# tensorflow/adanet

Measured on NVIDIA H100. Metric: candidate-train examples/sec per AdaNet iteration, higher is better.
Workload: dtype f32

## Files before the change

### adanet_b200/csrc/planes.cu

```cuda
#include <cuda.h>
#include <cudaTypedefs.h>

#include <stdlib.h>
#include <string.h>

#include <algorithm>
#include <atomic>
#include <mutex>
#include <string>
#include <unordered_map>
#include <vector>

#include "dense_simt.cuh"
#include "planes.cuh"
#include "wgmma.cuh"

namespace adn {
namespace pl {

static constexpr int BM = 128, BN = 64;
static constexpr int STAGES = 3;
static constexpr int A_TILE = BM * 128;
static constexpr int B_TILE = BN * 128;
static constexpr int STAGE_BYTES = 2 * A_TILE + 2 * B_TILE;
static constexpr int CONSUMERS = 2;
static constexpr int CONSUMER_WARPS = 4 * CONSUMERS;
static constexpr int EPI_WARPS = 4;
static constexpr int NUM_THREADS = 128 * (1 + CONSUMERS) + 32 * EPI_WARPS;
static constexpr int PRODUCER_REGS = 40, EPI_REGS = 136, CONSUMER_REGS = 168;
static_assert(128 * (PRODUCER_REGS + EPI_REGS) + 128 * CONSUMERS * CONSUMER_REGS <= 65536, "register file");
static_assert(PRODUCER_REGS < 65536 / NUM_THREADS && EPI_REGS > 65536 / NUM_THREADS &&
              CONSUMER_REGS > 65536 / NUM_THREADS, "setmaxnreg.dec / .inc");
static constexpr int ACC_BUFS = 2;
static constexpr int ACC_TILE_FLOATS = BM * BN;
static constexpr int ACC_BYTES = ACC_BUFS * ACC_TILE_FLOATS * 4;
static constexpr int EPI_STAGE_FLOATS = 32 * 16;
static constexpr int EPI_BYTES = EPI_WARPS * 2 * EPI_STAGE_FLOATS * 4;
static constexpr int BAR_BYTES = 256;
static constexpr int SMEM_BYTES = 1024 + STAGES * STAGE_BYTES + ACC_BYTES + EPI_BYTES + BAR_BYTES;
static_assert(SMEM_BYTES <= 232448, "shared memory per block");
static constexpr int MAX_SPLITS = 64;

template <int FMT> struct Fmt;
template <> struct Fmt<FMT_TF32> {
  static constexpr int BK = 32;
  static constexpr int CHUNK = 4;
};
template <> struct Fmt<FMT_F16> {
  static constexpr int BK = 64;
  static constexpr int CHUNK = 2;
};

enum { EPI_BIAS_ACT = 0, EPI_MASK = 1, EPI_PARTIAL = 2 };

struct GemmParams {
  int M, N;
  int tiles_m, tiles_n, splits;
  int tiles;
  float inv_tiles, inv_tiles_n, inv_tiles_m;
  int total_kb;
  int kb_per_split;
  int a_mn, b_mn;
  int out_planes;
  int m_fastest;
  void* out;
  void* out_lo;
  int ldc;
  int out_nb32;
  int out_tma;
  const float* bias;
  int act;
  uint32_t* out_bits;
  const uint32_t* mask_bits;
  float* colsum_part;
  int colsum_ld;
  float out_mul;
  unsigned int* ovf;
  uint32_t drop_thresh;
  uint32_t drop_key0;
  float drop_scale;
  const int64_t* drop_step;
};

__device__ __forceinline__ uint32_t smem_u32(const void* p) { return (uint32_t)__cvta_generic_to_shared(p); }

__device__ __forceinline__ void mbar_init(uint32_t bar, uint32_t count) {
  asm volatile("mbarrier.init.shared::cta.b64 [%0], %1;" ::"r"(bar), "r"(count));
}
__device__ __forceinline__ void mbar_expect_tx(uint32_t bar, uint32_t bytes) {
  asm volatile("mbarrier.arrive.expect_tx.shared::cta.b64 _, [%0], %1;" ::"r"(bar), "r"(bytes) : "memory");
}
__device__ __forceinline__ void mbar_arrive(uint32_t bar) {
  asm volatile("mbarrier.arrive.shared::cta.b64 _, [%0];" ::"r"(bar) : "memory");
}
__device__ __forceinline__ void mbar_wait(uint32_t bar, uint32_t parity) {
  uint32_t ok = 0;
  long long t0 = 0;
  for (uint32_t it = 0;; ++it) {
    asm volatile(
        "{\n\t.reg .pred p;\n\t"
        "mbarrier.try_wait.parity.shared::cta.b64 p, [%1], %2;\n\t"
        "selp.u32 %0, 1, 0, p;\n\t}"
        : "=r"(ok)
        : "r"(bar), "r"(parity)
        : "memory");
    if (ok) return;
    if ((it & 1023u) == 1023u) {
      long long now = clock64();
      if (t0 == 0) t0 = now;
      else if (now - t0 > 4000000000LL) __trap();
    }
  }
}
__device__ __forceinline__ void tma_load_3d(const CUtensorMap* map, uint32_t bar, uint32_t dst, int c0, int c1, int c2) {
  asm volatile(
      "cp.async.bulk.tensor.3d.shared::cluster.global.mbarrier::complete_tx::bytes [%0], [%1, {%3, %4, %5}], [%2];"
      ::"r"(dst), "l"(reinterpret_cast<uint64_t>(map)), "r"(bar), "r"(c0), "r"(c1), "r"(c2)
      : "memory");
}
__device__ __forceinline__ void tma_store_3d(const CUtensorMap* map, uint32_t src, int c0, int c1, int c2) {
  asm volatile("cp.async.bulk.tensor.3d.global.shared::cta.bulk_group [%0, {%2, %3, %4}], [%1];"
               ::"l"(reinterpret_cast<uint64_t>(map)), "r"(src), "r"(c0), "r"(c1), "r"(c2)
               : "memory");
}
__device__ __forceinline__ void bulk_commit() { asm volatile("cp.async.bulk.commit_group;" ::: "memory"); }
__device__ __forceinline__ void bulk_wait_read0() { asm volatile("cp.async.bulk.wait_group.read 0;" ::: "memory"); }
__device__ __forceinline__ void bulk_wait_read1() { asm volatile("cp.async.bulk.wait_group.read 1;" ::: "memory"); }
__device__ __forceinline__ void bulk_wait0() { asm volatile("cp.async.bulk.wait_group 0;" ::: "memory"); }
__device__ __forceinline__ void fence_async_smem() { asm volatile("fence.proxy.async.shared::cta;" ::: "memory"); }
__device__ __forceinline__ void sts_v4(uint32_t addr, uint32_t a, uint32_t b, uint32_t c, uint32_t d) {
  asm volatile("st.shared.v4.b32 [%0], {%1, %2, %3, %4};" ::"r"(addr), "r"(a), "r"(b), "r"(c), "r"(d) : "memory");
}
__device__ __forceinline__ void tma_prefetch_desc(const CUtensorMap* map) {
  asm volatile("prefetch.tensormap [%0];" ::"l"(reinterpret_cast<uint64_t>(map)) : "memory");
}

struct Item {
  int m0, n0, kb0, nkb, split;
};
__device__ __forceinline__ int fast_div(int n, float inv) { return (int)(((float)n + 0.5f) * inv); }

__device__ __forceinline__ Item decode_item(const GemmParams& g, int item) {
  Item it;
  it.split = (g.splits == 1) ? 0 : fast_div(item, g.inv_tiles);
  const int t = item - it.split * g.tiles;
  if (g.m_fastest) {
    const int tn = fast_div(t, g.inv_tiles_m);
    it.n0 = tn * BN;
    it.m0 = (t - tn * g.tiles_m) * BM;
  } else {
    const int tm = (g.tiles_n == 1) ? t : fast_div(t, g.inv_tiles_n);
    it.m0 = tm * BM;
    it.n0 = (t - tm * g.tiles_n) * BN;
  }
  it.kb0 = it.split * g.kb_per_split;
  it.nkb = min(g.total_kb, it.kb0 + g.kb_per_split) - it.kb0;
  return it;
}

__device__ __forceinline__ uint32_t pack_h2(__half a, __half b) {
  return (uint32_t)__half_as_ushort(a) | ((uint32_t)__half_as_ushort(b) << 16);
}

__device__ __forceinline__ void st_global_v8(void* p, const uint32_t (&w)[8]) {
  uint4* q = reinterpret_cast<uint4*>(p);
  q[0] = make_uint4(w[0], w[1], w[2], w[3]);
  q[1] = make_uint4(w[4], w[5], w[6], w[7]);
}

template <int FMT>
__device__ __forceinline__ void store_row32_planes(const GemmParams& g, const float* a, int my_row, int cbase) {
  constexpr int BK = Fmt<FMT>::BK;
  const size_t poff = ((size_t)(cbase / BK) * g.M + my_row) * BK + (cbase % BK);
  if (FMT == FMT_F16) {
    uint32_t hw[16], lw[16];
#pragma unroll
    for (int q = 0; q < 16; ++q) {
      const __half2 h2 = __floats2half2_rn(a[2 * q], a[2 * q + 1]);
      const float2 hf = __half22float2(h2);
      const __half2 l2 = __floats2half2_rn((a[2 * q] - hf.x) * 2048.0f, (a[2 * q + 1] - hf.y) * 2048.0f);
      hw[q] = *reinterpret_cast<const uint32_t*>(&h2);
      lw[q] = *reinterpret_cast<const uint32_t*>(&l2);
    }
    __half* hp = reinterpret_cast<__half*>(g.out) + poff;
    __half* lp = reinterpret_cast<__half*>(g.out_lo) + poff;
    st_global_v8(hp, reinterpret_cast<const uint32_t(&)[8]>(hw[0]));
    st_global_v8(hp + 16, reinterpret_cast<const uint32_t(&)[8]>(hw[8]));
    st_global_v8(lp, reinterpret_cast<const uint32_t(&)[8]>(lw[0]));
    st_global_v8(lp + 16, reinterpret_cast<const uint32_t(&)[8]>(lw[8]));
  } else {
    uint32_t hw[32], lw[32];
#pragma unroll
    for (int j = 0; j < 32; ++j) {
      float h, l;
// ... 244 lines not shown
              *reinterpret_cast<float4*>(op) = make_float4(v[0], v[1], v[2], v[3]);
            } else {
#pragma unroll
              for (int k = 0; k < 4; ++k)
                if (col + k < g.N) op[k] = v[k];
            }
          }
        }
      }
      if (EPI == EPI_MASK && g.colsum_part) {
#pragma unroll
        for (int k = 0; k < 4; ++k) {
          cs[k] += __shfl_xor_sync(0xffffffffu, cs[k], 4);
          cs[k] += __shfl_xor_sync(0xffffffffu, cs[k], 8);
          cs[k] += __shfl_xor_sync(0xffffffffu, cs[k], 16);
        }
        if (rsub == 0) {
          float* cp = g.colsum_part + (size_t)(mrow0 >> 5) * g.colsum_ld + col;
#pragma unroll
          for (int k = 0; k < 4; ++k)
            if (col + k < g.colsum_ld) cp[k] = cs[k];
        }
      }
    }
    __syncwarp();
  }
#undef ADN_SWZ
}

static constexpr int MAX_GROUP = 8;

struct alignas(64) Problem {
  CUtensorMap a_hi, a_lo, b_hi, b_lo;
  CUtensorMap o_hi, o_lo;
  GemmParams g;
  int item0;
  int pad_[3];
};
struct alignas(64) Group {
  Problem p[MAX_GROUP];
  int n;
  int total_items;
};

__device__ __forceinline__ int find_problem(const Group& grp, int cur, int item, int& next0) {
  while (item >= next0) {
    ++cur;
    next0 = (cur + 1 < grp.n) ? grp.p[cur + 1].item0 : 0x7fffffff;
  }
  return cur;
}
__device__ __forceinline__ int first_next0(const Group& grp) { return grp.n > 1 ? grp.p[1].item0 : 0x7fffffff; }

struct EpiItem {
  int p;
  Item it;
  uint32_t mw0, mw1;
  uint32_t drop_step;
};
template <int EPI>
__device__ __forceinline__ EpiItem epi_fetch(const Group& grp, int& cur, int& next0, int item, int tile_row) {
  EpiItem e;
  cur = find_problem(grp, cur, item, next0);
  e.p = cur;
  const GemmParams& g = grp.p[cur].g;
  e.it = decode_item(g, item - grp.p[cur].item0);
  e.mw0 = e.mw1 = 0xffffffffu;
  if (EPI == EPI_MASK && g.mask_bits) {
    const int my_row = e.it.m0 + tile_row, kbo = e.it.n0 >> 5;
    const bool row_ok = my_row < g.M;
    e.mw0 = (row_ok && kbo < g.out_nb32) ? __ldg(g.mask_bits + (size_t)kbo * g.M + my_row) : 0u;
    e.mw1 = (row_ok && kbo + 1 < g.out_nb32) ? __ldg(g.mask_bits + (size_t)(kbo + 1) * g.M + my_row) : 0u;
  }
  e.drop_step = (EPI == EPI_BIAS_ACT && g.drop_thresh != 0u) ? (uint32_t)(*g.drop_step) : 0u;
  return e;
}

template <int R> __device__ __forceinline__ void setmaxnreg_inc() { asm volatile("setmaxnreg.inc.sync.aligned.u32 %0;" ::"n"(R)); }
template <int R> __device__ __forceinline__ void setmaxnreg_dec() { asm volatile("setmaxnreg.dec.sync.aligned.u32 %0;" ::"n"(R)); }

__device__ __forceinline__ int acc_off(int row, int col) {
  return row * BN + ((((col >> 2) ^ row) & 7) | ((col >> 2) & 8)) * 4 + (col & 3);
}

template <int FMT>
__device__ __forceinline__ void fold_chunk(float (&acc)[32], const float (&H)[32], const float (&S)[32]) {
#pragma unroll
  for (int j = 0; j < 32; ++j) acc[j] += H[j];
  if (FMT == FMT_F16) {
#pragma unroll
    for (int j = 0; j < 32; ++j) acc[j] = fmaf(S[j], 1.0f / 2048.0f, acc[j]);
  } else {
#pragma unroll
    for (int j = 0; j < 32; ++j) acc[j] += S[j];
  }
}

template <int A_MN, int B_MN>
__device__ __forceinline__ void f16_kblock(uint32_t st, int wgi, float (&H)[32], float (&S)[32], bool first) {
  const uint32_t a_hi = st + (uint32_t)wgi * 8192u, a_lo = a_hi + A_TILE;
  const uint32_t b_hi = st + 2 * A_TILE, b_lo = b_hi + B_TILE;
  constexpr uint32_t a_step = A_MN ? 2048u : 32u, b_step = B_MN ? 2048u : 32u;
#pragma unroll
  for (int k = 0; k < 4; ++k) {
    const uint32_t sd = (first && k == 0) ? 0u : 1u;
    const uint64_t dah = wg::desc_sw128(a_hi + k * a_step), dal = wg::desc_sw128(a_lo + k * a_step);
    const uint64_t dbh = wg::desc_sw128(b_hi + k * b_step), dbl = wg::desc_sw128(b_lo + k * b_step);
    wg::mma_f16_n64<A_MN, B_MN>(H, dah, dbh, sd);
    wg::mma_f16_n64<A_MN, B_MN>(S, dah, dbl, sd);
    wg::mma_f16_n64<A_MN, B_MN>(S, dal, dbh, 1u);
  }
}

__device__ __forceinline__ uint32_t sw128_off(int r, int c) {
  return (uint32_t)(r * 128 + ((((c >> 4) ^ r) & 7) << 4) + (c & 15));
}
template <int MN>
__device__ __forceinline__ uint32_t tf32_off(int mn, int k) {
  return MN ? (uint32_t)((mn >> 5) * 4096) + sw128_off(k, 4 * (mn & 31)) : sw128_off(mn, 4 * k);
}
__device__ __forceinline__ void mma_tf32_16x8(float* d, const uint32_t (&a)[4], uint32_t b0, uint32_t b1) {
  asm volatile("mma.sync.aligned.m16n8k8.row.col.f32.tf32.tf32.f32 {%0, %1, %2, %3}, {%4, %5, %6, %7}, {%8, %9}, "
               "{%0, %1, %2, %3};"
               : "+f"(d[0]), "+f"(d[1]), "+f"(d[2]), "+f"(d[3])
               : "r"(a[0]), "r"(a[1]), "r"(a[2]), "r"(a[3]), "r"(b0), "r"(b1));
}
template <int A_MN, int B_MN>
__device__ __forceinline__ void tf32_kblock(const uint8_t* st, int arow0, int lane, float (&H)[32], float (&S)[32]) {
  const uint8_t* ah = st;
  const uint8_t* al = st + A_TILE;
  const uint8_t* bh = st + 2 * A_TILE;
  const uint8_t* bl = bh + B_TILE;
  const int gid = lane >> 2, tq = lane & 3;
#pragma unroll
  for (int ks = 0; ks < 4; ++ks) {
    uint32_t fa_h[4], fa_l[4];
#pragma unroll
    for (int e = 0; e < 4; ++e) {
      const uint32_t o = tf32_off<A_MN>(arow0 + gid + 8 * (e & 1), 8 * ks + tq + 4 * (e >> 1));
      fa_h[e] = *reinterpret_cast<const uint32_t*>(ah + o);
      fa_l[e] = *reinterpret_cast<const uint32_t*>(al + o);
    }
#pragma unroll
    for (int j = 0; j < 8; ++j) {
      const uint32_t o0 = tf32_off<B_MN>(8 * j + gid, 8 * ks + tq), o1 = tf32_off<B_MN>(8 * j + gid, 8 * ks + tq + 4);
      const uint32_t bh0 = *reinterpret_cast<const uint32_t*>(bh + o0), bh1 = *reinterpret_cast<const uint32_t*>(bh + o1);
      const uint32_t bl0 = *reinterpret_cast<const uint32_t*>(bl + o0), bl1 = *reinterpret_cast<const uint32_t*>(bl + o1);
      mma_tf32_16x8(&H[4 * j], fa_h, bh0, bh1);
      mma_tf32_16x8(&S[4 * j], fa_h, bl0, bl1);
      mma_tf32_16x8(&S[4 * j], fa_l, bh0, bh1);
    }
  }
}
template <int FMT, int EPI>
__global__ void __launch_bounds__(NUM_THREADS, 1)
pl_gemm_kernel(const __grid_constant__ Group grp) {
  constexpr int BK = Fmt<FMT>::BK;
  constexpr int CHUNK = Fmt<FMT>::CHUNK;
  constexpr int A_MN = EPI == EPI_PARTIAL, B_MN = EPI != EPI_MASK;
  extern __shared__ uint8_t smem_raw[];
  uint8_t* smem = reinterpret_cast<uint8_t*>((reinterpret_cast<uintptr_t>(smem_raw) + 1023) & ~(uintptr_t)1023);
  float* acc_stage = reinterpret_cast<float*>(smem + STAGES * STAGE_BYTES);
  float* epi_stage = reinterpret_cast<float*>(smem + STAGES * STAGE_BYTES + ACC_BYTES);
  uint64_t* bars = reinterpret_cast<uint64_t*>(smem + STAGES * STAGE_BYTES + ACC_BYTES + EPI_BYTES);
  uint64_t* full_bar = bars;
  uint64_t* empty_bar = bars + STAGES;
  uint64_t* tile_full = bars + 2 * STAGES;
  uint64_t* tile_empty = tile_full + ACC_BUFS;

  const int warp = __shfl_sync(0xffffffffu, threadIdx.x >> 5, 0);
  const int lane = threadIdx.x & 31;
  const int n_items = grp.total_items;

  if (threadIdx.x == 0) {
    for (int s = 0; s < STAGES; ++s) {
      mbar_init(smem_u32(&full_bar[s]), 1);
      mbar_init(smem_u32(&empty_bar[s]), CONSUMER_WARPS);
    }
    for (int b = 0; b < ACC_BUFS; ++b) {
      mbar_init(smem_u32(&tile_full[b]), 128 * CONSUMERS);
      mbar_init(smem_u32(&tile_empty[b]), 32 * EPI_WARPS);
    }
    asm volatile("fence.mbarrier_init.release.cluster;" ::: "memory");
  }
  if (warp == 1 && lane < grp.n) {
    tma_prefetch_desc(&grp.p[lane].a_hi);
    tma_prefetch_desc(&grp.p[lane].a_lo);
    tma_prefetch_desc(&grp.p[lane].b_hi);
    tma_prefetch_desc(&grp.p[lane].b_lo);
  }
  __syncthreads();

  if (warp < 4) {
    setmaxnreg_dec<PRODUCER_REGS>();
    if (warp == 0 && lane == 0) {
      uint32_t s = 0, ph = 0;
      int cur = 0, next0 = first_next0(grp);
      const uint32_t smem0 = smem_u32(smem);
      for (int item = blockIdx.x; item < n_items; item += gridDim.x) {
        cur = find_problem(grp, cur, item, next0);
        const Problem& pr = grp.p[cur];
        const GemmParams& g = pr.g;
        const Item it = decode_item(g, item - pr.item0);
        for (int kb = 0; kb < it.nkb; ++kb) {
          mbar_wait(smem_u32(&empty_bar[s]), ph ^ 1);
          const uint32_t fb = smem_u32(&full_bar[s]);
          mbar_expect_tx(fb, STAGE_BYTES);
          const uint32_t base = smem0 + s * STAGE_BYTES;
          const int kc = it.kb0 + kb;
          const int a1 = A_MN ? kc * BK : it.m0, a2 = A_MN ? (it.m0 / BK) : kc;
          const int b1 = B_MN ? kc * BK : it.n0, b2 = B_MN ? (it.n0 / BK) : kc;
          tma_load_3d(&pr.a_hi, fb, base, 0, a1, a2);
          tma_load_3d(&pr.a_lo, fb, base + A_TILE, 0, a1, a2);
          tma_load_3d(&pr.b_hi, fb, base + 2 * A_TILE, 0, b1, b2);
          tma_load_3d(&pr.b_lo, fb, base + 2 * A_TILE + B_TILE, 0, b1, b2);
          if (++s == STAGES) { s = 0; ph ^= 1; }
        }
      }
    }
    return;
  }

  if (warp >= 4 * (1 + CONSUMERS)) {
    setmaxnreg_inc<EPI_REGS>();
    const int ew = warp - 4 * (1 + CONSUMERS);
    float* stage = epi_stage + ew * 2 * EPI_STAGE_FLOATS;
    const int row = 32 * ew + lane;
    int cur = 0, next0 = first_next0(grp);
    EpiItem nx{};
    if ((int)blockIdx.x < n_items) nx = epi_fetch<EPI>(grp, cur, next0, blockIdx.x, row);
    uint32_t tcount = 0;
    for (int item = blockIdx.x; item < n_items; item += gridDim.x, ++tcount) {
      const EpiItem e = nx;
      if (item + (int)gridDim.x < n_items) nx = epi_fetch<EPI>(grp, cur, next0, item + gridDim.x, row);
      const GemmParams& g = grp.p[e.p].g;
      const Item& it = e.it;
      const uint32_t buf = tcount & 1u;
      mbar_wait(smem_u32(&tile_full[buf]), (tcount >> 1) & 1u);
      const float* tile = acc_stage + buf * ACC_TILE_FLOATS;
      const int mrow0 = it.m0 + 32 * ew;
      float* dense = reinterpret_cast<float*>(g.out);
      if (EPI == EPI_PARTIAL) dense += (size_t)it.split * g.M * g.N;
      const bool out_planes = g.out_planes != 0;
      const bool dense_vec = !out_planes && ((g.ldc & 3) == 0) && ((reinterpret_cast<uintptr_t>(dense) & 15) == 0);
      const int rows_ok = min(32, g.M - mrow0);
      const uint32_t mw0 = e.mw0, mw1 = e.mw1;
#pragma unroll 1
      for (int h = 0; h < 2; ++h) {
        const int cs = 32 * h;
        float acc[32];
#pragma unroll
        for (int q = 0; q < 8; ++q) {
          const float4 v = *reinterpret_cast<const float4*>(tile + acc_off(row, cs + 4 * q));
          acc[4 * q] = v.x; acc[4 * q + 1] = v.y; acc[4 * q + 2] = v.z; acc[4 * q + 3] = v.w;
        }
        if (h == 1) mbar_arrive(smem_u32(&tile_empty[buf]));
        const int ncol0 = it.n0 + cs;
        const uint32_t mw = h ? mw1 : mw0;
        if (FMT == FMT_F16 && !out_planes) {
          if (lane == 0) bulk_wait_read0();
          __syncwarp();
        }
        emit_slice<FMT, EPI>(g, out_planes, acc, mw, stage, lane, mrow0, ncol0, rows_ok, dense, dense_vec, true,
                             &grp.p[e.p].o_hi, &grp.p[e.p].o_lo, e.drop_step);
      }
    }
    if (FMT == FMT_F16 && lane == 0) bulk_wait0();
    return;
  }

  setmaxnreg_inc<CONSUMER_REGS>();
  const int wgi = warp / 4 - 1;
  const int wq = warp & 3;
  const int gid = lane >> 2, tq = lane & 3;
  const uint32_t smem0 = smem_u32(smem);
  uint32_t s = 0, ph = 0;
  int cur = 0, next0 = first_next0(grp);
  uint32_t tcount = 0;
  float H[32], S[32];
#pragma unroll
  for (int j = 0; j < 32; ++j) H[j] = S[j] = 0.f;
  for (int item = blockIdx.x; item < n_items; item += gridDim.x, ++tcount) {
    cur = find_problem(grp, cur, item, next0);
    const GemmParams& g = grp.p[cur].g;
    const Item it = decode_item(g, item - grp.p[cur].item0);
    float acc[32];
#pragma unroll
    for (int j = 0; j < 8; ++j)
#pragma unroll
      for (int e = 0; e < 4; ++e) {
        const int col = it.n0 + 8 * j + 2 * tq + (e & 1);
        acc[4 * j + e] = (EPI == EPI_BIAS_ACT && g.bias && col < g.N) ? __ldg(g.bias + col) : 0.f;
      }
    for (int kb = 0; kb < it.nkb; ++kb) {
      const bool first = (kb % CHUNK) == 0;
      const bool last = (kb % CHUNK) == CHUNK - 1 || kb == it.nkb - 1;
      mbar_wait(smem_u32(&full_bar[s]), ph);
      if (FMT == FMT_F16) {
        wg::fence_regs(H);
        wg::fence_regs(S);
        wg::fence();
        f16_kblock<A_MN, B_MN>(smem0 + s * STAGE_BYTES, wgi, H, S, first);
        wg::commit();
        wg::wait<0>();
        wg::fence_regs(H);
        wg::fence_regs(S);
      } else {
        if (first) {
#pragma unroll
          for (int j = 0; j < 32; ++j) H[j] = S[j] = 0.f;
        }
        tf32_kblock<A_MN, B_MN>(smem + s * STAGE_BYTES, 64 * wgi + 16 * wq, lane, H, S);
      }
      __syncwarp();
      if (lane == 0) mbar_arrive(smem_u32(&empty_bar[s]));
      if (++s == STAGES) { s = 0; ph ^= 1; }
      if (last) fold_chunk<FMT>(acc, H, S);
    }
    const uint32_t buf = tcount & 1u;
    mbar_wait(smem_u32(&tile_empty[buf]), ((tcount >> 1) & 1u) ^ 1u);
    float* tile = acc_stage + buf * ACC_TILE_FLOATS;
#pragma unroll
    for (int j = 0; j < 8; ++j) {
      const int row = 64 * wgi + 16 * wq + gid, col = 8 * j + 2 * tq;
      *reinterpret_cast<float2*>(tile + acc_off(row, col)) = make_float2(acc[4 * j], acc[4 * j + 1]);
      *reinterpret_cast<float2*>(tile + acc_off(row + 8, col)) = make_float2(acc[4 * j + 2], acc[4 * j + 3]);
    }
    mbar_arrive(smem_u32(&tile_full[buf]));
  }
}

template <int FMT>
__global__ void __launch_bounds__(256)
split_kernel(const float* __restrict__ src, void* __restrict__ hi_, void* __restrict__ lo_, uint32_t* __restrict__ bits,
             int rows, int cols, int nkb, float scale, unsigned int* ovf) {
  constexpr int BK = Fmt<FMT>::BK;
  const int vec_per_row = nkb * (BK / 4);
  const int64_t nvec = (int64_t)rows * vec_per_row;
  const int64_t nvec_pad = (nvec + 31) & ~(int64_t)31;
  const bool vec_src = ((cols & 3) == 0) && ((reinterpret_cast<uintptr_t>(src) & 15) == 0);
  bool over = false;
  for (int64_t i = (int64_t)blockIdx.x * blockDim.x + threadIdx.x; i < nvec_pad; i += (int64_t)gridDim.x * blockDim.x) {
    const bool live = i < nvec;
    const int r = live ? (int)(i / vec_per_row) : 0;
    const int c = live ? (int)(i % vec_per_row) * 4 : 0;
    float v[4] = {0.f, 0.f, 0.f, 0.f};
    if (live) {
      if (vec_src && c + 3 < cols) {
        float4 t = __ldg(reinterpret_cast<const float4*>(src + (size_t)r * cols + c));
        v[0] = t.x; v[1] = t.y; v[2] = t.z; v[3] = t.w;
      } else {
#pragma unroll
        for (int q = 0; q < 4; ++q) v[q] = (c + q < cols) ? __ldg(src + (size_t)r * cols + c + q) : 0.f;
      }
#pragma unroll
      for (int q = 0; q < 4; ++q) v[q] *= scale;
    }
    uint32_t nib = 0u;
#pragma unroll
    for (int q = 0; q < 4; ++q) nib |= (v[q] > 0.f) ? (1u << q) : 0u;
    uint32_t w = nib << (4 * (threadIdx.x & 7));
    w |= __shfl_xor_sync(0xffffffffu, w, 1);
    w |= __shfl_xor_sync(0xffffffffu, w, 2);
    w |= __shfl_xor_sync(0xffffffffu, w, 4);
    if (live) {
      const size_t dst = ((size_t)(c / BK) * rows + r) * BK + (c % BK);
      if (FMT == FMT_F16) {
        __half h[4], l[4];
#pragma unroll
        for (int q = 0; q < 4; ++q) {
          split_f16(v[q], h[q], l[q]);
          over |= f16_overflows(v[q]);
        }
        *reinterpret_cast<uint2*>(reinterpret_cast<__half*>(hi_) + dst) = make_uint2(pack_h2(h[0], h[1]), pack_h2(h[2], h[3]));
        *reinterpret_cast<uint2*>(reinterpret_cast<__half*>(lo_) + dst) = make_uint2(pack_h2(l[0], l[1]), pack_h2(l[2], l[3]));
      } else {
        float h[4], l[4];
#pragma unroll
        for (int q = 0; q < 4; ++q) split_tf32(v[q], h[q], l[q]);
        *reinterpret_cast<float4*>(reinterpret_cast<float*>(hi_) + dst) = make_float4(h[0], h[1], h[2], h[3]);
        *reinterpret_cast<float4*>(reinterpret_cast<float*>(lo_) + dst) = make_float4(l[0], l[1], l[2], l[3]);
      }
      if ((threadIdx.x & 7) == 0) bits[(size_t)(c >> 5) * rows + r] = w;
    }
  }
  if (over) raise_overflow(ovf);
}

template <int FMT>
__global__ void __launch_bounds__(256)
merge_kernel(const void* __restrict__ hi_, const void* __restrict__ lo_, float* __restrict__ dst, int rows, int cols, int nkb) {
  constexpr int BK = Fmt<FMT>::BK;
  const int64_t n = (int64_t)rows * nkb * BK;
  for (int64_t i = (int64_t)blockIdx.x * blockDim.x + threadIdx.x; i < n; i += (int64_t)gridDim.x * blockDim.x) {
    const int cb = (int)(i % BK);
    const int64_t t = i / BK;
    const int r = (int)(t % rows);
    const int c = (int)(t / rows) * BK + cb;
    if (c < cols) {
      if (FMT == FMT_F16)
        dst[(size_t)r * cols + c] = merge_f16(reinterpret_cast<const __half*>(hi_)[i], reinterpret_cast<const __half*>(lo_)[i]);
      else
        dst[(size_t)r * cols + c] = reinterpret_cast<const float*>(hi_)[i] + reinterpret_cast<const float*>(lo_)[i];
    }
  }
}

__device__ unsigned int g_plane_overflow = 0u;

static PFN_cuTensorMapEncodeTiled g_encode = nullptr;
static unsigned int* g_ovf_addr = nullptr;
static std::atomic<int> g_format{-1};

int format() {
  int f = g_format.load();
  if (f >= 0) return f;
  const char* e = getenv("ADN_PLANES");
  f = (e && (!strcmp(e, "tf32") || !strcmp(e, "TF32"))) ? FMT_TF32 : FMT_F16;
  g_format.store(f);
  return f;
}
int set_format(int fmt) {
  if (fmt != FMT_TF32 && fmt != FMT_F16) return fail(ADN_ERR_INVALID, "adn_set_plane_format: bad format %d", fmt);
  g_format.store(fmt);
  return ADN_OK;
}
unsigned int* overflow_flag() { return g_ovf_addr; }

int read_overflow(int* out_host, int reset, cudaStream_t st) {
  if (!g_ovf_addr) return fail(ADN_ERR_CUDA, "pl: adn_init() was not called");
  unsigned int v = 0;
  ADN_CUDA(cudaMemcpyAsync(&v, g_ovf_addr, sizeof(v), cudaMemcpyDeviceToHost, st));
  if (reset) ADN_CUDA(cudaMemsetAsync(g_ovf_addr, 0, sizeof(v), st));
  ADN_CUDA(cudaStreamSynchronize(st));
  *out_host = (int)v;
  return ADN_OK;
}

int init() {
  static std::once_flag once;
  static int rc = ADN_OK;
  std::call_once(once, []() {
    void* fn = nullptr;
    cudaDriverEntryPointQueryResult q;
    cudaError_t e = cudaGetDriverEntryPoint("cuTensorMapEncodeTiled", &fn, cudaEnableDefault, &q);
    if (e != cudaSuccess || q != cudaDriverEntryPointSuccess || fn == nullptr) {
      (void)cudaGetLastError();
      rc = fail(ADN_ERR_CUDA, "pl::init: cuTensorMapEncodeTiled entry point unavailable");
      return;
    }
    g_encode = reinterpret_cast<PFN_cuTensorMapEncodeTiled>(fn);
    bool ok = true;
#define ADN_PL_ATTR(F, E) \
  ok = ok && (cudaFuncSetAttribute(pl_gemm_kernel<F, E>, cudaFuncAttributeMaxDynamicSharedMemorySize, SMEM_BYTES) == cudaSuccess)
    ADN_PL_ATTR(FMT_TF32, EPI_BIAS_ACT); ADN_PL_ATTR(FMT_TF32, EPI_MASK); ADN_PL_ATTR(FMT_TF32, EPI_PARTIAL);
    ADN_PL_ATTR(FMT_F16, EPI_BIAS_ACT); ADN_PL_ATTR(FMT_F16, EPI_MASK); ADN_PL_ATTR(FMT_F16, EPI_PARTIAL);
#undef ADN_PL_ATTR
    if (!ok) {
      (void)cudaGetLastError();
      rc = fail(ADN_ERR_CUDA, "pl::init: cudaFuncSetAttribute(smem=%d) failed", SMEM_BYTES);
      return;
    }
    void* addr = nullptr;
    if (cudaGetSymbolAddress(&addr, g_plane_overflow) != cudaSuccess || !addr) {
      (void)cudaGetLastError();
      rc = fail(ADN_ERR_CUDA, "pl::init: cudaGetSymbolAddress(g_plane_overflow) failed");
      return;
    }
    g_ovf_addr = reinterpret_cast<unsigned int*>(addr);
  });
  return rc;
}

int64_t planes_bytes_fmt(int fmt, int64_t rows, int64_t cols) { return planes_bytes(fmt, rows, cols); }

struct Operand {
  const void* hi;
  const void* lo;
  int64_t rows, nkb;
  int mn_major;
};
static Operand operand(int fmt, const void* planes, int64_t rows, int64_t cols, int mn_major) {
  const char* p = reinterpret_cast<const char*>(planes);
  return Operand{p, p + plane_bytes1(fmt, rows, cols), rows, ceil_div(cols, fmt_bk(fmt)), mn_major};
}

struct MapKey {
  const void* ptr;
  int64_t rows, nkb;
  int mn, fmt;
  int box = 0;
  bool operator==(const MapKey& o) const {
    return ptr == o.ptr && rows == o.rows && nkb == o.nkb && mn == o.mn && fmt == o.fmt && box == o.box;
  }
};
struct MapKeyHash {
  size_t operator()(const MapKey& k) const {
    size_t h = reinterpret_cast<uintptr_t>(k.ptr) * 0x9E3779B97F4A7C15ull;
    h ^= (size_t)k.rows * 0xC2B2AE3D27D4EB4Full + ((size_t)k.nkb << 20) + ((size_t)k.mn << 1) + (size_t)k.fmt + ((size_t)k.box << 40);
    return h ^ (h >> 29);
  }
};
static std::mutex g_map_mu;
static std::unordered_map<MapKey, CUtensorMap, MapKeyHash> g_maps;
static std::atomic<long long> g_map_hits{0}, g_map_misses{0};
long long map_cache_hits() { return g_map_hits.load(); }
long long map_cache_misses() { return g_map_misses.load(); }

static int make_map(int fmt, CUtensorMap* map, const void* plane, int64_t rows, int64_t nkb, int mn_major, int box) {
  if (!g_encode) return fail(ADN_ERR_CUDA, "pl: adn_init() was not called");
  const MapKey key{plane, rows, nkb, mn_major, fmt, box};
  {
    std::lock_guard<std::mutex> lk(g_map_mu);
    auto it = g_maps.find(key);
    if (it != g_maps.end()) {
      *map = it->second;
      g_map_hits.fetch_add(1, std::memory_order_relaxed);
      return ADN_OK;
    }
  }
  const int bk = fmt_bk(fmt), es = fmt_esize(fmt);
  cuuint64_t gdim[3] = {(cuuint64_t)bk, (cuuint64_t)rows, (cuuint64_t)nkb};
  cuuint64_t gstride[2] = {(cuuint64_t)bk * es, (cuuint64_t)rows * bk * es};
  cuuint32_t box_k[3] = {(cuuint32_t)bk, (cuuint32_t)box, 1u};
  cuuint32_t box_mn[3] = {(cuuint32_t)bk, (cuuint32_t)bk, (cuuint32_t)(box / bk)};
  cuuint32_t estr[3] = {1u, 1u, 1u};
  const CUtensorMapSwizzle sw = CU_TENSOR_MAP_SWIZZLE_128B;
  CUresult r = g_encode(map, fmt == FMT_F16 ? CU_TENSOR_MAP_DATA_TYPE_FLOAT16 : CU_TENSOR_MAP_DATA_TYPE_FLOAT32, 3,
                        const_cast<void*>(plane), gdim, gstride, mn_major ? box_mn : box_k, estr,
                        CU_TENSOR_MAP_INTERLEAVE_NONE, sw, CU_TENSOR_MAP_L2_PROMOTION_L2_256B,
                        CU_TENSOR_MAP_FLOAT_OOB_FILL_NONE);
  if (r != CUDA_SUCCESS) return fail(ADN_ERR_CUDA, "cuTensorMapEncodeTiled failed (%d) rows=%lld nkb=%lld mn=%d fmt=%d", (int)r,
                                     (long long)rows, (long long)nkb, mn_major, fmt);
  g_map_misses.fetch_add(1, std::memory_order_relaxed);
  std::lock_guard<std::mutex> lk(g_map_mu);
  if (g_maps.size() > 16384) g_maps.clear();
  g_maps.emplace(key, *map);
  return ADN_OK;
}

static int make_store_map(CUtensorMap* map, const void* plane, int64_t rows, int64_t nkb) {
  if (!g_encode) return fail(ADN_ERR_CUDA, "pl: adn_init() was not called");
  const MapKey key{plane, rows, nkb, 2, FMT_F16};
  {
    std::lock_guard<std::mutex> lk(g_map_mu);
    auto it = g_maps.find(key);
    if (it != g_maps.end()) {
      *map = it->second;
      g_map_hits.fetch_add(1, std::memory_order_relaxed);
      return ADN_OK;
    }
  }
  cuuint64_t gdim[3] = {64u, (cuuint64_t)rows, (cuuint64_t)nkb};
  cuuint64_t gstride[2] = {128u, (cuuint64_t)rows * 128u};
  cuuint32_t box[3] = {32u, 32u, 1u};
  cuuint32_t estr[3] = {1u, 1u, 1u};
  CUresult r = g_encode(map, CU_TENSOR_MAP_DATA_TYPE_FLOAT16, 3, const_cast<void*>(plane), gdim, gstride, box, estr,
                        CU_TENSOR_MAP_INTERLEAVE_NONE, CU_TENSOR_MAP_SWIZZLE_64B, CU_TENSOR_MAP_L2_PROMOTION_NONE,
                        CU_TENSOR_MAP_FLOAT_OOB_FILL_NONE);
  if (r != CUDA_SUCCESS) return fail(ADN_ERR_CUDA, "cuTensorMapEncodeTiled (store box) failed (%d) rows=%lld nkb=%lld", (int)r,
                                     (long long)rows, (long long)nkb);
  g_map_misses.fetch_add(1, std::memory_order_relaxed);
  std::lock_guard<std::mutex> lk(g_map_mu);
  if (g_maps.size() > 16384) g_maps.clear();
  g_maps.emplace(key, *map);
  return ADN_OK;
}
static int store_mode() {
  static const int env = getenv("ADN_PL_TMA_STORE") ? atoi(getenv("ADN_PL_TMA_STORE")) : 1;
  return env;
}

struct GemmDesc {
  Operand a, b;
  GemmParams g;
};

static int encode_maps(int fmt, const GemmDesc& d, CUtensorMap* a_hi, CUtensorMap* a_lo, CUtensorMap* b_hi, CUtensorMap* b_lo,
                       const char* what) {
  if ((reinterpret_cast<uintptr_t>(d.a.hi) | reinterpret_cast<uintptr_t>(d.a.lo) | reinterpret_cast<uintptr_t>(d.b.hi) |
       reinterpret_cast<uintptr_t>(d.b.lo)) & 127)
    return fail(ADN_ERR_INVALID, "%s: plane buffers must be 256 B aligned", what);
  int rc;
  if ((rc = make_map(fmt, a_hi, d.a.hi, d.a.rows, d.a.nkb, d.a.mn_major, BM))) return rc;
  if ((rc = make_map(fmt, a_lo, d.a.lo, d.a.rows, d.a.nkb, d.a.mn_major, BM))) return rc;
  if ((rc = make_map(fmt, b_hi, d.b.hi, d.b.rows, d.b.nkb, d.b.mn_major, BN))) return rc;
  if ((rc = make_map(fmt, b_lo, d.b.lo, d.b.rows, d.b.nkb, d.b.mn_major, BN))) return rc;
  return ADN_OK;
}

static int item_order_m_fastest(const GemmParams& g) {
  static const int env = getenv("ADN_PL_MFAST") ? atoi(getenv("ADN_PL_MFAST")) : -1;
  if (env >= 0) return env;
  (void)g;
  return 0;
}

template <int FMT, int EPI>
static void launch_kernel(const Group& grp, int grid, cudaStream_t st) {
  pl_gemm_kernel<FMT, EPI><<<grid, NUM_THREADS, SMEM_BYTES, st>>>(grp);
}
template <int EPI>
static int launch_group(int fmt, const GemmDesc* d, int n, cudaStream_t st, const char* what) {
  {
    for (int i0 = 0; i0 < n; i0 += MAX_GROUP) {
      const int m = std::min(MAX_GROUP, n - i0);
      Group grp;
      memset(&grp, 0, sizeof(grp));
      int items = 0;
      for (int i = 0; i < m; ++i) {
        const GemmDesc& src = d[i0 + i];
        Problem& pr = grp.p[i];
        if (src.a.mn_major != (EPI == EPI_PARTIAL) || src.b.mn_major != (EPI != EPI_MASK))
          return fail(ADN_ERR_INVALID, "%s: operand majorness does not match the epilogue kind", what);
        int rc = encode_maps(fmt, src, &pr.a_hi, &pr.a_lo, &pr.b_hi, &pr.b_lo, what);
        if (rc) return rc;
        pr.g = src.g;
        pr.g.out_tma = 0;
        if (fmt == FMT_F16 && EPI != EPI_PARTIAL && src.g.out_planes && store_mode() && (src.g.out_nb32 & 1) == 0 &&
            ((reinterpret_cast<uintptr_t>(src.g.out) | reinterpret_cast<uintptr_t>(src.g.out_lo)) & 127) == 0) {
          if ((rc = make_store_map(&pr.o_hi, src.g.out, src.g.M, src.g.out_nb32 / 2))) return rc;
          if ((rc = make_store_map(&pr.o_lo, src.g.out_lo, src.g.M, src.g.out_nb32 / 2))) return rc;
          pr.g.out_tma = 1;
        }
        pr.g.a_mn = src.a.mn_major;
        pr.g.b_mn = src.b.mn_major;
        pr.g.tiles_m = (int)ceil_div(pr.g.M, BM);
        pr.g.tiles_n = (int)ceil_div(pr.g.N, BN);
        pr.g.tiles = pr.g.tiles_m * pr.g.tiles_n;
        if ((int64_t)pr.g.tiles * pr.g.splits >= (1 << 21))
          return fail(ADN_ERR_UNSUPPORTED, "%s: %d work items exceed the decode range", what, pr.g.tiles * pr.g.splits);
        pr.g.inv_tiles = 1.0f / (float)pr.g.tiles;
        pr.g.inv_tiles_n = 1.0f / (float)pr.g.tiles_n;
        pr.g.inv_tiles_m = 1.0f / (float)pr.g.tiles_m;
        pr.g.m_fastest = item_order_m_fastest(pr.g);
        pr.g.ovf = g_ovf_addr;
        pr.item0 = items;
        items += pr.g.tiles_m * pr.g.tiles_n * pr.g.splits;
      }
      grp.n = m;
      grp.total_items = items;
      const int grid = std::min(items, sm_count());
      if (fmt == FMT_F16) launch_kernel<FMT_F16, EPI>(grp, grid, st);
      else launch_kernel<FMT_TF32, EPI>(grp, grid, st);
      ADN_CHECK_LAUNCH(what);
    }
  }
  return ADN_OK;
}

int split(int fmt, const float* src, int64_t rows, int64_t cols, void* planes, int log2_scale, cudaStream_t st) {
  const int bk = fmt_bk(fmt);
  const int64_t nkb = ceil_div(cols, bk);
  const int64_t nvec = rows * nkb * (bk / 4);
  const int blocks = (int)std::max<int64_t>(1, std::min<int64_t>(ceil_div(nvec, 256), (int64_t)sm_count() * 16));
  const PlaneView v = plane_view(fmt, planes, rows, cols);
  const float scale = ldexpf(1.0f, log2_scale);
  if (fmt == FMT_F16)
    split_kernel<FMT_F16><<<blocks, 256, 0, st>>>(src, v.hi, v.lo, v.bits, (int)rows, (int)cols, (int)nkb, scale, g_ovf_addr);
  else
    split_kernel<FMT_TF32><<<blocks, 256, 0, st>>>(src, v.hi, v.lo, v.bits, (int)rows, (int)cols, (int)nkb, scale, g_ovf_addr);
  ADN_CHECK_LAUNCH("planes split");
  return ADN_OK;
}

int merge(int fmt, const void* planes, int64_t rows, int64_t cols, float* dst, cudaStream_t st) {
  const int bk = fmt_bk(fmt);
  const int64_t nkb = ceil_div(cols, bk);
  const int64_t n = rows * nkb * bk;
  const int blocks = (int)std::max<int64_t>(1, std::min<int64_t>(ceil_div(n, 256), (int64_t)sm_count() * 16));
  const PlaneView v = plane_view(fmt, const_cast<void*>(planes), rows, cols);
  if (fmt == FMT_F16) merge_kernel<FMT_F16><<<blocks, 256, 0, st>>>(v.hi, v.lo, dst, (int)rows, (int)cols, (int)nkb);
  else merge_kernel<FMT_TF32><<<blocks, 256, 0, st>>>(v.hi, v.lo, dst, (int)rows, (int)cols, (int)nkb);
  ADN_CHECK_LAUNCH("planes merge");
  return ADN_OK;
}

static int max_dw_splits(int64_t in, int64_t out) {
  int64_t s = (16LL << 20) / std::max<int64_t>(1, in * out);
  if (s > MAX_SPLITS) s = MAX_SPLITS;
  if (s < 1) s = 1;
  return (int)s;
}

int64_t dense_bwd_workspace_bytes(int64_t batch, int64_t in, int64_t out) {
  int64_t b = align_up((int64_t)max_dw_splits(in, out) * in * out * (int64_t)sizeof(float), 256);
  b += align_up(ceil_div(batch, 32) * in * (int64_t)sizeof(float), 256);
  b += align_up(64 * in * (int64_t)sizeof(float), 256);
  return b + 512;
}

int dense_fwd_group(int fmt, const FwdOp* ops, int n, int64_t batch, cudaStream_t st) {
  if (n <= 0) return ADN_OK;
  const int bk = fmt_bk(fmt);
  std::vector<GemmDesc> d((size_t)n);
  for (int i = 0; i < n; ++i) {
    const FwdOp& o = ops[i];
    GemmDesc& e = d[(size_t)i];
    e.a = operand(fmt, o.xp, batch, o.in, 0);
    e.b = operand(fmt, o.wp, o.in, o.out, 1);
    GemmParams g{};
    g.M = (int)batch; g.N = (int)o.out;
    g.total_kb = (int)ceil_div(o.in, bk); g.kb_per_split = g.total_kb; g.splits = 1;
    g.bias = o.bias; g.act = o.act;
    g.out_mul = 1.0f;
    if (o.dropout_rate > 0.f) {
      if (!o.yp || !o.dropout_step) return fail(ADN_ERR_INVALID, "pl dense_fwd: dropout needs planes out and a step counter");
      const double t = (double)o.dropout_rate * 4294967296.0;
      g.drop_thresh = t >= 4294967295.0 ? 0xffffffffu : (uint32_t)t;
      if (g.drop_thresh == 0u) g.drop_thresh = 1u;
      g.drop_key0 = o.dropout_seed * 0x9E3779B1u + (uint32_t)o.dropout_layer * 0x85EBCA77u + 0x27D4EB2Fu;
      g.drop_scale = 1.0f / (1.0f - o.dropout_rate);
      g.drop_step = o.dropout_step;
    }
    if (o.yp) {
      const PlaneView v = plane_view(fmt, o.yp, batch, o.out);
      g.out_planes = 1;
      g.out = v.hi; g.out_lo = v.lo; g.out_nb32 = (int)bits_blocks(fmt, o.out);
      g.out_bits = v.bits;
    } else {
      g.out = o.y; g.ldc = (int)o.out;
    }
    e.g = g;
  }
  return launch_group<EPI_BIAS_ACT>(fmt, d.data(), n, st, "pl dense_fwd gemm");
}

int dense_bwd_group(int fmt, const BwdOp* ops, int n, int64_t batch, cudaStream_t st) {
  if (n <= 0) return ADN_OK;
  const int bk = fmt_bk(fmt);
  const int workers = sm_count();
  struct Carve { float* part; float* cspart; float* cspart2; int splits; };
  std::vector<Carve> cv((size_t)n);
  std::vector<GemmDesc> dwd, dxd;
  const int64_t kb_b = ceil_div(batch, bk);
  int64_t best_kps = kb_b;
  {
    static std::mutex mu;
    static std::unordered_map<std::string, int64_t> memo;
    std::string key = std::to_string(batch) + ":" + std::to_string(fmt);
    for (int i = 0; i < n; ++i)
      if (ops[i].dw) key += "," + std::to_string(ops[i].in) + "x" + std::to_string(ops[i].out);
    bool hit = false;
    {
      std::lock_guard<std::mutex> lk(mu);
      auto it = memo.find(key);
      if (it != memo.end()) { best_kps = it->second; hit = true; }
    }
    if (!hit) {
      const double kItemOverhead = 6.0;
      const double kReduceKbPerByte = 1.0 / (2.5e6 * 0.4);
      double best_t = 1e30;
      std::vector<double> load((size_t)workers);
      int64_t last_kps = -1;
      for (int s0 = 1; s0 <= MAX_SPLITS && s0 <= kb_b; ++s0) {
        const int64_t kps = ceil_div(kb_b, s0);
        if (kps == last_kps) continue;
        last_kps = kps;
        std::fill(load.begin(), load.end(), 0.0);
        int64_t item = 0;
        double reduce_bytes = 0.0;
        bool any = false;
        for (int i = 0; i < n; ++i) {
          if (!ops[i].dw) continue;
          any = true;
          const int64_t k_i = std::max<int64_t>(kps, ceil_div(kb_b, max_dw_splits(ops[i].in, ops[i].out)));
          const int64_t s_i = ceil_div(kb_b, k_i);
          const int64_t tiles = ceil_div(ops[i].in, BM) * ceil_div(ops[i].out, BN);
          for (int64_t sp = 0; sp < s_i; ++sp) {
            const double kb_item = (double)(std::min(kb_b, (sp + 1) * k_i) - sp * k_i);
            for (int64_t t = 0; t < tiles; ++t, ++item) load[(size_t)(item % workers)] += kb_item + kItemOverhead;
          }
          if (s_i > 1) reduce_bytes += (double)(s_i + 1) * (double)ops[i].in * (double)ops[i].out * 4.0;
        }
        if (!any) break;
        const double t = *std::max_element(load.begin(), load.end()) +
                         reduce_bytes * kReduceKbPerByte + (reduce_bytes > 0 ? 10.0 : 0.0);
        if (t < best_t) { best_t = t; best_kps = kps; }
      }
      std::lock_guard<std::mutex> lk(mu);
      if (memo.size() > 4096) memo.clear();
      memo[key] = best_kps;
    }
  }
  for (int i = 0; i < n; ++i) {
    const BwdOp& o = ops[i];
    if (!o.ws || o.ws_bytes < dense_bwd_workspace_bytes(batch, o.in, o.out))
      return fail(ADN_ERR_WORKSPACE, "pl dense_bwd: op %d workspace %lld < %lld bytes", i, (long long)o.ws_bytes,
                  (long long)dense_bwd_workspace_bytes(batch, o.in, o.out));
    const float unscale = ldexpf(1.0f, -o.dz_log2_scale);
    char* p = reinterpret_cast<char*>((reinterpret_cast<uintptr_t>(o.ws) + 255) & ~(uintptr_t)255);
    const int max_s = max_dw_splits(o.in, o.out);
    Carve& c = cv[(size_t)i];
    c.part = reinterpret_cast<float*>(p);
    p += align_up((int64_t)max_s * o.in * o.out * (int64_t)sizeof(float), 256);
    c.cspart = reinterpret_cast<float*>(p);
    p += align_up(ceil_div(batch, 32) * o.in * (int64_t)sizeof(float), 256);
// ... 78 lines not shown
```

Measured before the change: 7.340 million.

## Add thin-K GEMM kernel variant with two epilogue groups and lighter consumers

Adds a THIN kernel configuration used for f16 non-partial GEMMs whose K fits within one fold chunk. It uses two pipeline stages, two epilogue warpgroups that alternate tiles, and fewer consumer registers, and it skips the per-chunk fold by combining the hi and scaled lo accumulators directly with the bias at the end. The goal is to overlap the epilogue better on short-K GEMMs, where the epilogue dominates. The tradeoff is a different register and shared-memory balance and another kernel template to maintain.

```diff
diff --git a/adanet_b200/csrc/planes.cu b/adanet_b200/csrc/planes.cu
--- a/adanet_b200/csrc/planes.cu
+++ b/adanet_b200/csrc/planes.cu
@@ -19,27 +19,32 @@
 namespace pl {
 
 static constexpr int BM = 128, BN = 64;
-static constexpr int STAGES = 3;
 static constexpr int A_TILE = BM * 128;
 static constexpr int B_TILE = BN * 128;
 static constexpr int STAGE_BYTES = 2 * A_TILE + 2 * B_TILE;
 static constexpr int CONSUMERS = 2;
 static constexpr int CONSUMER_WARPS = 4 * CONSUMERS;
-static constexpr int EPI_WARPS = 4;
-static constexpr int NUM_THREADS = 128 * (1 + CONSUMERS) + 32 * EPI_WARPS;
-static constexpr int PRODUCER_REGS = 40, EPI_REGS = 136, CONSUMER_REGS = 168;
-static_assert(128 * (PRODUCER_REGS + EPI_REGS) + 128 * CONSUMERS * CONSUMER_REGS <= 65536, "register file");
-static_assert(PRODUCER_REGS < 65536 / NUM_THREADS && EPI_REGS > 65536 / NUM_THREADS &&
-              CONSUMER_REGS > 65536 / NUM_THREADS, "setmaxnreg.dec / .inc");
 static constexpr int ACC_BUFS = 2;
 static constexpr int ACC_TILE_FLOATS = BM * BN;
 static constexpr int ACC_BYTES = ACC_BUFS * ACC_TILE_FLOATS * 4;
 static constexpr int EPI_STAGE_FLOATS = 32 * 16;
-static constexpr int EPI_BYTES = EPI_WARPS * 2 * EPI_STAGE_FLOATS * 4;
 static constexpr int BAR_BYTES = 256;
-static constexpr int SMEM_BYTES = 1024 + STAGES * STAGE_BYTES + ACC_BYTES + EPI_BYTES + BAR_BYTES;
-static_assert(SMEM_BYTES <= 232448, "shared memory per block");
 static constexpr int MAX_SPLITS = 64;
+
+template <bool THIN> struct Cfg {
+  static constexpr int STAGES = THIN ? 2 : 3;
+  static constexpr int EPI_GROUPS = THIN ? 2 : 1;
+  static constexpr int EPI_WARPS = 4 * EPI_GROUPS;
+  static constexpr int NUM_THREADS = 128 * (1 + CONSUMERS + EPI_GROUPS);
+  static constexpr int PRODUCER_REGS = 40, CONSUMER_REGS = THIN ? 96 : 168, EPI_REGS = THIN ? 120 : 136;
+  static constexpr int ENTRY_REGS = 65536 / NUM_THREADS / 8 * 8;
+  static_assert(128 * PRODUCER_REGS + 128 * CONSUMERS * CONSUMER_REGS + 128 * EPI_GROUPS * EPI_REGS <=
+                NUM_THREADS * ENTRY_REGS, "register file");
+  static_assert(PRODUCER_REGS < ENTRY_REGS && EPI_REGS > ENTRY_REGS && CONSUMER_REGS >= ENTRY_REGS, "setmaxnreg.dec / .inc");
+  static constexpr int EPI_BYTES = EPI_WARPS * 2 * EPI_STAGE_FLOATS * 4;
+  static constexpr int SMEM_BYTES = 1024 + STAGES * STAGE_BYTES + ACC_BYTES + EPI_BYTES + BAR_BYTES;
+  static_assert(SMEM_BYTES <= 232448, "shared memory per block");
+};
 
 template <int FMT> struct Fmt;
 template <> struct Fmt<FMT_TF32> {
@@ -590,17 +595,19 @@
     }
   }
 }
-template <int FMT, int EPI>
-__global__ void __launch_bounds__(NUM_THREADS, 1)
+template <int FMT, int EPI, bool THIN>
+__global__ void __launch_bounds__(Cfg<THIN>::NUM_THREADS, 1)
 pl_gemm_kernel(const __grid_constant__ Group grp) {
+  using C = Cfg<THIN>;
   constexpr int BK = Fmt<FMT>::BK;
   constexpr int CHUNK = Fmt<FMT>::CHUNK;
+  constexpr int STAGES = C::STAGES;
   constexpr int A_MN = EPI == EPI_PARTIAL, B_MN = EPI != EPI_MASK;
   extern __shared__ uint8_t smem_raw[];
   uint8_t* smem = reinterpret_cast<uint8_t*>((reinterpret_cast<uintptr_t>(smem_raw) + 1023) & ~(uintptr_t)1023);
   float* acc_stage = reinterpret_cast<float*>(smem + STAGES * STAGE_BYTES);
   float* epi_stage = reinterpret_cast<float*>(smem + STAGES * STAGE_BYTES + ACC_BYTES);
-  uint64_t* bars = reinterpret_cast<uint64_t*>(smem + STAGES * STAGE_BYTES + ACC_BYTES + EPI_BYTES);
+  uint64_t* bars = reinterpret_cast<uint64_t*>(smem + STAGES * STAGE_BYTES + ACC_BYTES + C::EPI_BYTES);
   uint64_t* full_bar = bars;
   uint64_t* empty_bar = bars + STAGES;
   uint64_t* tile_full = bars + 2 * STAGES;
@@ -617,7 +624,7 @@
     }
     for (int b = 0; b < ACC_BUFS; ++b) {
       mbar_init(smem_u32(&tile_full[b]), 128 * CONSUMERS);
-      mbar_init(smem_u32(&tile_empty[b]), 32 * EPI_WARPS);
+      mbar_init(smem_u32(&tile_empty[b]), 128);
     }
     asm volatile("fence.mbarrier_init.release.cluster;" ::: "memory");
   }
@@ -630,7 +637,7 @@
   __syncthreads();
 
   if (warp < 4) {
-    setmaxnreg_dec<PRODUCER_REGS>();
+    setmaxnreg_dec<C::PRODUCER_REGS>();
     if (warp == 0 && lane == 0) {
       uint32_t s = 0, ph = 0;
       int cur = 0, next0 = first_next0(grp);
@@ -659,18 +666,19 @@
     return;
   }
 
-  if (warp >= 4 * (1 + CONSUMERS)) {
-    setmaxnreg_inc<EPI_REGS>();
-    const int ew = warp - 4 * (1 + CONSUMERS);
-    float* stage = epi_stage + ew * 2 * EPI_STAGE_FLOATS;
+  auto epilogue = [&]() {
+    setmaxnreg_inc<C::EPI_REGS>();
+    const int ew = warp & 3, eg = C::EPI_GROUPS == 1 ? 0 : warp / 4 - (1 + CONSUMERS);
+    float* stage = epi_stage + (warp - 4 * (1 + CONSUMERS)) * 2 * EPI_STAGE_FLOATS;
     const int row = 32 * ew + lane;
+    const int item0 = blockIdx.x + eg * gridDim.x, stride = C::EPI_GROUPS * gridDim.x;
     int cur = 0, next0 = first_next0(grp);
     EpiItem nx{};
-    if ((int)blockIdx.x < n_items) nx = epi_fetch<EPI>(grp, cur, next0, blockIdx.x, row);
-    uint32_t tcount = 0;
-    for (int item = blockIdx.x; item < n_items; item += gridDim.x, ++tcount) {
+    if (item0 < n_items) nx = epi_fetch<EPI>(grp, cur, next0, item0, row);
+    uint32_t tcount = eg;
+    for (int item = item0; item < n_items; item += stride, tcount += C::EPI_GROUPS) {
       const EpiItem e = nx;
-      if (item + (int)gridDim.x < n_items) nx = epi_fetch<EPI>(grp, cur, next0, item + gridDim.x, row);
+      if (item + stride < n_items) nx = epi_fetch<EPI>(grp, cur, next0, item + stride, row);
       const GemmParams& g = grp.p[e.p].g;
       const Item& it = e.it;
       const uint32_t buf = tcount & 1u;
@@ -704,67 +712,96 @@
       }
     }
     if (FMT == FMT_F16 && lane == 0) bulk_wait0();
-    return;
-  }
-
-  setmaxnreg_inc<CONSUMER_REGS>();
-  const int wgi = warp / 4 - 1;
-  const int wq = warp & 3;
-  const int gid = lane >> 2, tq = lane & 3;
-  const uint32_t smem0 = smem_u32(smem);
-  uint32_t s = 0, ph = 0;
-  int cur = 0, next0 = first_next0(grp);
-  uint32_t tcount = 0;
-  float H[32], S[32];
-#pragma unroll
-  for (int j = 0; j < 32; ++j) H[j] = S[j] = 0.f;
-  for (int item = blockIdx.x; item < n_items; item += gridDim.x, ++tcount) {
-    cur = find_problem(grp, cur, item, next0);
-    const GemmParams& g = grp.p[cur].g;
-    const Item it = decode_item(g, item - grp.p[cur].item0);
-    float acc[32];
-#pragma unroll
-    for (int j = 0; j < 8; ++j)
-#pragma unroll
-      for (int e = 0; e < 4; ++e) {
-        const int col = it.n0 + 8 * j + 2 * tq + (e & 1);
-        acc[4 * j + e] = (EPI == EPI_BIAS_ACT && g.bias && col < g.N) ? __ldg(g.bias + col) : 0.f;
-      }
-    for (int kb = 0; kb < it.nkb; ++kb) {
-      const bool first = (kb % CHUNK) == 0;
-      const bool last = (kb % CHUNK) == CHUNK - 1 || kb == it.nkb - 1;
-      mbar_wait(smem_u32(&full_bar[s]), ph);
-      if (FMT == FMT_F16) {
-        wg::fence_regs(H);
-        wg::fence_regs(S);
-        wg::fence();
-        f16_kblock<A_MN, B_MN>(smem0 + s * STAGE_BYTES, wgi, H, S, first);
-        wg::commit();
-        wg::wait<0>();
-        wg::fence_regs(H);
-        wg::fence_regs(S);
-      } else {
-        if (first) {
-#pragma unroll
-          for (int j = 0; j < 32; ++j) H[j] = S[j] = 0.f;
+  };
+
+  auto consumers = [&]() {
+    setmaxnreg_inc<C::CONSUMER_REGS>();
+    const int wgi = warp / 4 - 1;
+    const int wq = warp & 3;
+    const int gid = lane >> 2, tq = lane & 3;
+    const uint32_t smem0 = smem_u32(smem);
+    uint32_t s = 0, ph = 0;
+    int cur = 0, next0 = first_next0(grp);
+    uint32_t tcount = 0;
+    float H[32], S[32];
+#pragma unroll
+    for (int j = 0; j < 32; ++j) H[j] = S[j] = 0.f;
+    for (int item = blockIdx.x; item < n_items; item += gridDim.x, ++tcount) {
+      cur = find_problem(grp, cur, item, next0);
+      const GemmParams& g = grp.p[cur].g;
+      const Item it = decode_item(g, item - grp.p[cur].item0);
+      float acc[32];
+      if (!THIN) {
+#pragma unroll
+        for (int j = 0; j < 8; ++j)
+#pragma unroll
+          for (int e = 0; e < 4; ++e) {
+            const int col = it.n0 + 8 * j + 2 * tq + (e & 1);
+            acc[4 * j + e] = (EPI == EPI_BIAS_ACT && g.bias && col < g.N) ? __ldg(g.bias + col) : 0.f;
+          }
+      }
+      for (int kb = 0; kb < it.nkb; ++kb) {
+        const bool first = (kb % CHUNK) == 0;
+        const bool last = (kb % CHUNK) == CHUNK - 1 || kb == it.nkb - 1;
+        mbar_wait(smem_u32(&full_bar[s]), ph);
+        if (FMT == FMT_F16) {
+          wg::fence_regs(H);
+          wg::fence_regs(S);
+          wg::fence();
+          f16_kblock<A_MN, B_MN>(smem0 + s * STAGE_BYTES, wgi, H, S, first);
+          wg::commit();
+          wg::wait<0>();
+          wg::fence_regs(H);
+          wg::fence_regs(S);
+        } else {
+          if (first) {
+#pragma unroll
+            for (int j = 0; j < 32; ++j) H[j] = S[j] = 0.f;
+          }
+          tf32_kblock<A_MN, B_MN>(smem + s * STAGE_BYTES, 64 * wgi + 16 * wq, lane, H, S);
         }
-        tf32_kblock<A_MN, B_MN>(smem + s * STAGE_BYTES, 64 * wgi + 16 * wq, lane, H, S);
-      }
-      __syncwarp();
-      if (lane == 0) mbar_arrive(smem_u32(&empty_bar[s]));
-      if (++s == STAGES) { s = 0; ph ^= 1; }
-      if (last) fold_chunk<FMT>(acc, H, S);
-    }
-    const uint32_t buf = tcount & 1u;
-    mbar_wait(smem_u32(&tile_empty[buf]), ((tcount >> 1) & 1u) ^ 1u);
-    float* tile = acc_stage + buf * ACC_TILE_FLOATS;
-#pragma unroll
-    for (int j = 0; j < 8; ++j) {
-      const int row = 64 * wgi + 16 * wq + gid, col = 8 * j + 2 * tq;
-      *reinterpret_cast<float2*>(tile + acc_off(row, col)) = make_float2(acc[4 * j], acc[4 * j + 1]);
-      *reinterpret_cast<float2*>(tile + acc_off(row + 8, col)) = make_float2(acc[4 * j + 2], acc[4 * j + 3]);
-    }
-    mbar_arrive(smem_u32(&tile_full[buf]));
+        __syncwarp();
+        if (lane == 0) mbar_arrive(smem_u32(&empty_bar[s]));
+        if (++s == STAGES) { s = 0; ph ^= 1; }
+        if (!THIN && last) fold_chunk<FMT>(acc, H, S);
+      }
+      if (THIN) {
+#pragma unroll
+        for (int j = 0; j < 8; ++j)
+#pragma unroll
+          for (int e = 0; e < 4; ++e) {
+            const int col = it.n0 + 8 * j + 2 * tq + (e & 1);
+            H[4 * j + e] = ((EPI == EPI_BIAS_ACT && g.bias && col < g.N) ? __ldg(g.bias + col) : 0.f) + H[4 * j + e];
+          }
+#pragma unroll
+        for (int j = 0; j < 32; ++j) H[j] = fmaf(S[j], 1.0f / 2048.0f, H[j]);
+      }
+      const float (&res)[32] = THIN ? H : acc;
+      const uint32_t buf = tcount & 1u;
+      mbar_wait(smem_u32(&tile_empty[buf]), ((tcount >> 1) & 1u) ^ 1u);
+      float* tile = acc_stage + buf * ACC_TILE_FLOATS;
+#pragma unroll
+      for (int j = 0; j < 8; ++j) {
+        const int row = 64 * wgi + 16 * wq + gid, col = 8 * j + 2 * tq;
+        *reinterpret_cast<float2*>(tile + acc_off(row, col)) = make_float2(res[4 * j], res[4 * j + 1]);
+        *reinterpret_cast<float2*>(tile + acc_off(row + 8, col)) = make_float2(res[4 * j + 2], res[4 * j + 3]);
+      }
+      mbar_arrive(smem_u32(&tile_full[buf]));
+    }
+  };
+
+  if constexpr (THIN) {
+    if (warp < 4 * (1 + CONSUMERS)) {
+      consumers();
+      return;
+    }
+    epilogue();
+  } else {
+    if (warp >= 4 * (1 + CONSUMERS)) {
+      epilogue();
+      return;
+    }
+    consumers();
   }
 }
 
@@ -889,14 +926,17 @@
     }
     g_encode = reinterpret_cast<PFN_cuTensorMapEncodeTiled>(fn);
     bool ok = true;
-#define ADN_PL_ATTR(F, E) \
-  ok = ok && (cudaFuncSetAttribute(pl_gemm_kernel<F, E>, cudaFuncAttributeMaxDynamicSharedMemorySize, SMEM_BYTES) == cudaSuccess)
-    ADN_PL_ATTR(FMT_TF32, EPI_BIAS_ACT); ADN_PL_ATTR(FMT_TF32, EPI_MASK); ADN_PL_ATTR(FMT_TF32, EPI_PARTIAL);
-    ADN_PL_ATTR(FMT_F16, EPI_BIAS_ACT); ADN_PL_ATTR(FMT_F16, EPI_MASK); ADN_PL_ATTR(FMT_F16, EPI_PARTIAL);
+#define ADN_PL_ATTR(F, E, T)                                                                                   \
+  ok = ok && (cudaFuncSetAttribute(pl_gemm_kernel<F, E, T>, cudaFuncAttributeMaxDynamicSharedMemorySize,       \
+                                   Cfg<T>::SMEM_BYTES) == cudaSuccess)
+    ADN_PL_ATTR(FMT_TF32, EPI_BIAS_ACT, false); ADN_PL_ATTR(FMT_TF32, EPI_MASK, false); ADN_PL_ATTR(FMT_TF32, EPI_PARTIAL, false);
+    ADN_PL_ATTR(FMT_F16, EPI_BIAS_ACT, false); ADN_PL_ATTR(FMT_F16, EPI_MASK, false); ADN_PL_ATTR(FMT_F16, EPI_PARTIAL, false);
+    ADN_PL_ATTR(FMT_F16, EPI_BIAS_ACT, true); ADN_PL_ATTR(FMT_F16, EPI_MASK, true);
 #undef ADN_PL_ATTR
     if (!ok) {
       (void)cudaGetLastError();
-      rc = fail(ADN_ERR_CUDA, "pl::init: cudaFuncSetAttribute(smem=%d) failed", SMEM_BYTES);
+      rc = fail(ADN_ERR_CUDA, "pl::init: cudaFuncSetAttribute(smem=%d / %d) failed", Cfg<false>::SMEM_BYTES,
+                Cfg<true>::SMEM_BYTES);
       return;
     }
     void* addr = nullptr;
@@ -1034,9 +1074,14 @@
   return 0;
 }
 
-template <int FMT, int EPI>
+static int thin_mode() {
+  static const int env = getenv("ADN_PL_THIN") ? atoi(getenv("ADN_PL_THIN")) : 1;
+  return env;
+}
+
+template <int FMT, int EPI, bool THIN>
 static void launch_kernel(const Group& grp, int grid, cudaStream_t st) {
-  pl_gemm_kernel<FMT, EPI><<<grid, NUM_THREADS, SMEM_BYTES, st>>>(grp);
+  pl_gemm_kernel<FMT, EPI, THIN><<<grid, Cfg<THIN>::NUM_THREADS, Cfg<THIN>::SMEM_BYTES, st>>>(grp);
 }
 template <int EPI>
 static int launch_group(int fmt, const GemmDesc* d, int n, cudaStream_t st, const char* what) {
@@ -1046,6 +1091,7 @@
       Group grp;
       memset(&grp, 0, sizeof(grp));
       int items = 0;
+      bool thin = fmt == FMT_F16 && EPI != EPI_PARTIAL && thin_mode();
       for (int i = 0; i < m; ++i) {
         const GemmDesc& src = d[i0 + i];
         Problem& pr = grp.p[i];
@@ -1075,12 +1121,14 @@
         pr.g.ovf = g_ovf_addr;
         pr.item0 = items;
         items += pr.g.tiles_m * pr.g.tiles_n * pr.g.splits;
+        thin = thin && pr.g.total_kb <= Fmt<FMT_F16>::CHUNK;
       }
       grp.n = m;
       grp.total_items = items;
       const int grid = std::min(items, sm_count());
-      if (fmt == FMT_F16) launch_kernel<FMT_F16, EPI>(grp, grid, st);
-      else launch_kernel<FMT_TF32, EPI>(grp, grid, st);
+      if (fmt == FMT_TF32) launch_kernel<FMT_TF32, EPI, false>(grp, grid, st);
+      else if (!thin) launch_kernel<FMT_F16, EPI, false>(grp, grid, st);
+      else if constexpr (EPI != EPI_PARTIAL) launch_kernel<FMT_F16, EPI, true>(grp, grid, st);
       ADN_CHECK_LAUNCH(what);
     }
   }
```

Result: faster. 7.543 million (median of 6 runs) (+2.8%).
